# Spandan7724/Audio-Watermarking-Deep-Learning-Watermarks-for-Authenticating-Speech

Measured on AMD Instinct MI355X. Metric: 1-s@16kHz clips/sec (gen+det+loss fwd-bwd), higher is better.
Workload: dtype f32; 1 GPU; main16 train step: Generator+Detector+6 losses fwd-bwd + Adam, B=256 clips/GPU x 1 GPU, 1-s @ 16 kHz, message_bits=16 (BASELINE configs[2]); batch_per_gpu=256, global_batch=256, clip_len=16000, optimizer=fused flat Adam (wm_adam_step), parallelism=single

## Files before the change

audio-watermarking-deep-learning-watermarks-for-authenticating-speech_amd/csrc/lstm.hip:

```cpp
#include "wm_common.hpp"
#include <type_traits>
using namespace wm;

namespace {

#ifdef WM_STAMP
__device__ unsigned long long* g_lstm_stamp = nullptr;
#define LSTAMP(var, val) unsigned long long var; asm volatile("s_memtime %0\n\ts_waitcnt lgkmcnt(0)" : "=s"(var), "+v"(val))
#define LSTAMP_ACC(i, a, b) tm[i] += (b) - (a)
#else
#define LSTAMP(var, val)
#define LSTAMP_ACC(i, a, b)
#endif

__device__ __forceinline__ int gate_row(int np) { return (np & 3) * 64 + (np >> 2); }

typedef float v2f __attribute__((ext_vector_type(2)));
template <int K>
__device__ __forceinline__ float quad_bcast(float v) {
    constexpr int ctrl = K | (K << 2) | (K << 4) | (K << 6);
    return __int_as_float(__builtin_amdgcn_update_dpp(0, __float_as_int(v), ctrl, 0xf, 0xf, false));
}

__global__ __launch_bounds__(256) void lstm_xproj_kernel(const float* __restrict__ x, const float* __restrict__ w_ih,
// ... 613 lines not shown
#endif
    auto run_chunk = [&](const Buf& f, int t1) {
#pragma unroll
        for (int jj = 0; jj < CH; ++jj) {
            const int j = CH - 1 - jj, t = t1 - jj;
            if (t >= 0) {
                LSTAMP(ls0, dc);
                const float4 p = *reinterpret_cast<const float4*>(&part[pb][u][0]);
                const float act = f.ga[j];
                const float gi = quad_bcast<0>(act), gf = quad_bcast<1>(act), gg = quad_bcast<2>(act), go = quad_bcast<3>(act);
                const float tc = tanh_s(f.cc[j + 1]);
                const float cprev = (t >= 1) ? f.cc[j] : 0.f;
                const float S = is0 ? gg : (is1 ? cprev : (is2 ? gi : tc));
                const float D = is2 ? fmaf(-act, act, 1.f) : act * (1.f - act);
                const float M = S * D;
                const float K = go * fmaf(-tc, tc, 1.f);
                float dht = f.dh[j] + ((p.x + p.y) + (p.z + p.w));
                LSTAMP(ls1, dht);
                const float dct = fmaf(dht, K, dc);
                float da = (is3 ? dht : dct) * M;
                dc = dct * gf;
                LSTAMP(ls2, da);
                buf_store(sgb, da, vgb, (unsigned)t * 1024u);
                float Dd[4];
                rows_replicate(da, Dd);
                float psum = dot64_rowbcast(Dd, wt);
                LSTAMP(ls3, psum);
                part[pb ^ 1][lane][wave] = psum;
                pb ^= 1;
                LSTAMP(ls4, psum);
                __syncthreads();
                LSTAMP(ls5, dc);
                LSTAMP_ACC(0, ls0, ls1); LSTAMP_ACC(1, ls1, ls2); LSTAMP_ACC(2, ls2, ls3); LSTAMP_ACC(3, ls3, ls4); LSTAMP_ACC(4, ls4, ls5);
            }
        }
    };
    prefetch(A, T - 1);
    __syncthreads();
    for (int t1 = T - 1; t1 >= 0; t1 -= 2 * CH) {
        prefetch(Bf, t1 - CH);
        run_chunk(A, t1);
        prefetch(A, t1 - 2 * CH);
        run_chunk(Bf, t1 - CH);
    }
#ifdef WM_STAMP
    if (g_lstm_stamp && lane == 0) {
        unsigned long long* d = g_lstm_stamp + ((size_t)blockIdx.x * 4 + wave) * 6;
#pragma unroll
        for (int i = 0; i < 6; ++i) d[i] = tm[i];
    }
#endif
}

__global__ __launch_bounds__(512) void lstm_bwd_ws_kernel(float* __restrict__ gates, const float* __restrict__ cst,
                                                          const float* __restrict__ dh_out, const float* __restrict__ w_hh,
                                                          const float* __restrict__ x, const float* __restrict__ hseq,
                                                          float* __restrict__ partial, int T) {
    constexpr int CT = 32, PT = 36;
    extern __shared__ __align__(16) unsigned char smem_raw[];
    float* daT = reinterpret_cast<float*>(smem_raw);
    float (*part)[64][4] = reinterpret_cast<float (*)[64][4]>(daT + 2 * 256 * PT);
    const int b = blockIdx.x, tid = threadIdx.x, lane = tid & 63;
    const int wave = __builtin_amdgcn_readfirstlane(tid >> 6);
    float* out = partial + (size_t)b * (256 * 128 + 256);
    if (wave < 4) {
        __builtin_amdgcn_s_setprio(3);
        const int q = lane & 3, ul = lane >> 2, u = wave * 16 + ul, np = wave * 64 + lane;
        float wt[64];
#pragma unroll
        for (int j = 0; j < 64; ++j) wt[j] = w_hh[((j & 3) * 64 + wave * 16 + (j >> 2)) * 64 + lane];
        if (tid < 512 / 4) reinterpret_cast<float4*>(&part[0][0][0])[tid] = make_float4(0.f, 0.f, 0.f, 0.f);
        float dc = 0.f, dbs = 0.f;
        const wm_srd_t sgb = make_srd(gates + (size_t)b * T * 256, (size_t)T * 256 * sizeof(float));
        const wm_srd_t scb = make_srd(cst + (size_t)b * T * 64, (size_t)T * 64 * sizeof(float));
        const wm_srd_t sdh = make_srd(dh_out + (size_t)b * 64 * T, (size_t)64 * T * sizeof(float));
        const unsigned vgb = (unsigned)np * 4u, vcb = (unsigned)u * 4u, vdh = (unsigned)(u * T) * 4u;
        constexpr int CH = 8;
        struct Buf { float ga[CH], cc[CH + 1], dh[CH]; };
        Buf A, Bf;
        auto prefetch = [&](Buf& f, int t1) {
#pragma unroll
            for (int j = 0; j < CH; ++j) {
                const int t = max(t1 - CH + 1 + j, 0);
                f.ga[j] = buf_load(sgb, vgb, (unsigned)t * 1024u);
                f.dh[j] = buf_load(sdh, vdh, (unsigned)t * 4u);
            }
#pragma unroll
            for (int j = 0; j <= CH; ++j) f.cc[j] = buf_load(scb, vcb, (unsigned)max(t1 - CH + j, 0) * 256u);
        };
        const bool is0 = q == 0, is1 = q == 1, is2 = q == 2, is3 = q == 3;
        int pb = 0;
        auto run_chunk = [&](const Buf& f, int t1) {
            float dav[CH];
#pragma unroll
            for (int jj = 0; jj < CH; ++jj) {
                const int j = CH - 1 - jj, t = t1 - jj;
                const float4 p = *reinterpret_cast<const float4*>(&part[pb][u][0]);
                const float act = f.ga[j];
                const float gi = quad_bcast<0>(act), gf = quad_bcast<1>(act), gg = quad_bcast<2>(act), go = quad_bcast<3>(act);
                const float tc = tanh_s(f.cc[j + 1]);
                const float cprev = (t >= 1) ? f.cc[j] : 0.f;
                const float S = is0 ? gg : (is1 ? cprev : (is2 ? gi : tc));
                const float D = is2 ? fmaf(-act, act, 1.f) : act * (1.f - act);
                const float M = S * D;
                const float K = go * fmaf(-tc, tc, 1.f);
                const float dht = f.dh[j] + ((p.x + p.y) + (p.z + p.w));
                const float dct = fmaf(dht, K, dc);
                const float da = (is3 ? dht : dct) * M;
                dc = dct * gf;
                dav[j] = da;
                buf_store(sgb, da, vgb, (unsigned)t * 1024u);
                float Dd[4];
                rows_replicate(da, Dd);
                const float psum = dot64_rowbcast(Dd, wt);
                part[pb ^ 1][lane][wave] = psum;
                pb ^= 1;
                if (jj == CH - 1) {
                    const int t0 = t1 - (CH - 1);
                    float* d = daT + (((t0 >> 5) & 1) * 256 + np) * PT + (t0 & (CT - 1));
                    *reinterpret_cast<float4*>(d) = make_float4(dav[0], dav[1], dav[2], dav[3]);
                    *reinterpret_cast<float4*>(d + 4) = make_float4(dav[4], dav[5], dav[6], dav[7]);
                }
                dbs += da;
                __syncthreads();
            }
        };
        prefetch(A, T - 1);
        __syncthreads();
        for (int t1 = T - 1; t1 >= 0; t1 -= 2 * CH) {
            prefetch(Bf, t1 - CH);
            run_chunk(A, t1);
            prefetch(A, t1 - 2 * CH);
            run_chunk(Bf, t1 - CH);
        }
        out[256 * 128 + np] = dbs;
        return;
    }
    const int hw = wave - 4, half = lane >> 5, l31 = lane & 31;
    f32x16 acc[2][2][2];
#pragma unroll
    for (int i = 0; i < 8; ++i)
#pragma unroll
        for (int r = 0; r < 16; ++r) acc[i >> 2][(i >> 1) & 1][i & 1][r] = 0.f;
    const wm_srd_t sx = make_srd(x + (size_t)b * 64 * T, (size_t)64 * T * sizeof(float));
    const wm_srd_t sh = make_srd(hseq + (size_t)b * 64 * T, (size_t)64 * T * sizeof(float));
    float raw[8];
    auto load_raw = [&](int chunk, int u_) {
        const int ks = u_ >> 2, z = (u_ >> 1) & 1, ct = u_ & 1;
        const unsigned v = (unsigned)((32 * ct + l31) * T + 8 * half) * 4u;
        const int ts = chunk * CT + 16 * ks;
        if (z == 0) {
            const f32x4 a0 = buf_load4(sx, v, (unsigned)ts * 4u), a1 = buf_load4(sx, v, (unsigned)(ts + 4) * 4u);
            raw[0] = a0[0]; raw[1] = a0[1]; raw[2] = a0[2]; raw[3] = a0[3]; raw[4] = a1[0]; raw[5] = a1[1]; raw[6] = a1[2]; raw[7] = a1[3];
        } else {
#pragma unroll
            for (int e = 0; e < 8; ++e) {
                const int te = ts + e - 1;
                const float r_ = buf_load(sh, te < 0 ? v - 4u : v, (unsigned)max(te, 0) * 4u);
                raw[e] = (te < 0 && half == 0) ? 0.f : r_;
            }
        }
    };
    auto split8 = [&](const float (&v)[8], bf16x8 (&P)[3]) {
        unsigned w_[3][4];
#pragma unroll
        for (int i = 0; i < 4; ++i) split3_pair(v[2 * i], v[2 * i + 1], w_[0][i], w_[1][i], w_[2][i]);
#pragma unroll
        for (int p = 0; p < 3; ++p) P[p] = __builtin_bit_cast(bf16x8, make_uint4(w_[p][0], w_[p][1], w_[p][2], w_[p][3]));
    };
    bf16x8 Af[2][3], Bp[3];
    auto slot = [&](int chunk, int sl) {
        const int u_ = sl >> 2, k = sl & 3, ks = u_ >> 2, z = (u_ >> 1) & 1, ct = u_ & 1;
        if (k == 0) {
            if ((u_ & 3) == 0) {
#pragma unroll
                for (int rt = 0; rt < 2; ++rt) {
                    const float* src = daT + ((chunk & 1) * 256 + 64 * hw + 32 * rt + l31) * PT + 16 * ks + 8 * half;
                    const float4 a0 = *reinterpret_cast<const float4*>(src), a1 = *reinterpret_cast<const float4*>(src + 4);
                    const float v[8] = {a0.x, a0.y, a0.z, a0.w, a1.x, a1.y, a1.z, a1.w};
                    split8(v, Af[rt]);
                }
            }
            split8(raw, Bp);
            if (u_ < 7) load_raw(chunk, u_ + 1); else load_raw(max(chunk - 1, 0), 0);
            return;
        }
        constexpr int PA[6] = {1, 0, 2, 0, 1, 0}, PB[6] = {1, 2, 0, 1, 0, 0};
#pragma unroll
        for (int i = 0; i < 4; ++i) {
            const int m = 4 * (k - 1) + i, rt = m / 6, j = m % 6;
            acc[z][rt][ct] = __builtin_amdgcn_mfma_f32_32x32x16_bf16(Af[rt][PA[j]], Bp[PB[j]], acc[z][rt][ct], 0, 0, 0);
        }
    };
    const int nch = T / CT;
    load_raw(nch - 1, 0);
    __syncthreads();
    for (int c = nch - 1; c >= 0; --c) {
        const bool work = c + 1 < nch;
#pragma unroll
        for (int sl = 0; sl < CT; ++sl) {
            if (work) slot(c + 1, sl);
            __syncthreads();
        }
    }
#pragma unroll
    for (int sl = 0; sl < CT; ++sl) slot(0, sl);
#pragma unroll
    for (int z = 0; z < 2; ++z)
#pragma unroll
        for (int rt = 0; rt < 2; ++rt)
#pragma unroll
            for (int ct = 0; ct < 2; ++ct)
#pragma unroll
                for (int r = 0; r < 16; ++r)
                    out[(64 * hw + 32 * rt + mfma_row(r, half)) * 128 + 64 * z + 32 * ct + l31] = acc[z][rt][ct][r];
}

__global__ __launch_bounds__(256) void lstm_bwd_fused_kernel(float* __restrict__ gates, const float* __restrict__ cst,
                                                             const float* __restrict__ dh_out, const float* __restrict__ w_hh,
                                                             const float* __restrict__ w_ih, float* __restrict__ dx, int T) {
    constexpr int HS = WM_LSTM_HS, CHK = 32, PITCH = 72, NP = 3, PDP = 33;
    constexpr int DIMG = NP * CHK * PITCH;
    extern __shared__ __align__(16) unsigned char smem_raw[];
    unsigned short* Dab = reinterpret_cast<unsigned short*>(smem_raw);
    float* Pd = reinterpret_cast<float*>(Dab + 2 * 4 * DIMG);
    float* das = Pd + 4 * 64 * PDP;
    float* part = das + 4 * 64;
    const int b = blockIdx.x, tid = threadIdx.x, lane = tid & 63, wave = tid >> 6, half = lane >> 5, l31 = lane & 31;
    const int q = lane & 3, ul = lane >> 2, u = wave * 16 + ul, np = wave * 64 + lane;
    v2f wt[32];
#pragma unroll
    for (int j = 0; j < 64; j += 2)
        wt[j / 2] = v2f{w_hh[((j & 3) * 64 + wave * 16 + (j >> 2)) * 64 + lane],
                        w_hh[(((j + 1) & 3) * 64 + wave * 16 + ((j + 1) >> 2)) * 64 + lane]};
    bf16x8 Wt[2][4][NP];
#pragma unroll
    for (int mt = 0; mt < 2; ++mt)
#pragma unroll
        for (int ks = 0; ks < 4; ++ks) {
            float v[8];
#pragma unroll
            for (int j = 0; j < 8; ++j) v[j] = w_ih[gate_row(wave * 64 + 16 * ks + 8 * half + j) * 64 + mt * 32 + l31];
            unsigned a[4], m[4], l[4];
#pragma unroll
            for (int j = 0; j < 4; ++j) split3_pair(v[2 * j], v[2 * j + 1], a[j], m[j], l[j]);
            Wt[mt][ks][0] = __builtin_bit_cast(bf16x8, make_uint4(a[0], a[1], a[2], a[3]));
            Wt[mt][ks][1] = __builtin_bit_cast(bf16x8, make_uint4(m[0], m[1], m[2], m[3]));
            Wt[mt][ks][2] = __builtin_bit_cast(bf16x8, make_uint4(l[0], l[1], l[2], l[3]));
        }
    if (tid < 128) reinterpret_cast<float4*>(part)[tid] = make_float4(0.f, 0.f, 0.f, 0.f);
    float dc = 0.f;
    float* gb = gates + (size_t)b * T * 256 + np;
    const float* cb = cst + (size_t)b * T * 64 + u;
    const float* dhb = dh_out + ((size_t)b * 64 + u) * T;

    constexpr int CH = 8;
    struct Buf { float ga[CH], cc[CH + 1], dh[CH]; };
    Buf A, Bf;
    auto prefetch = [&](Buf& f, int t1) {
// ... 541 lines not shown
    if (g_lstm_fwd_ws) {
        static wm::DevOnce donew[2];
        if (int rc = wm::lds_opt_in(reinterpret_cast<const void*>(lstm_fwd_ws_kernel<true>), lds, donew[0])) return rc;
        if (int rc = wm::lds_opt_in(reinterpret_cast<const void*>(lstm_fwd_ws_kernel<false>), lds, donew[1])) return rc;
        if (gates && cst) hipLaunchKernelGGL(lstm_fwd_ws_kernel<true>, dim3(B), dim3(512), lds, stream, x, w_ih, b_ih, b_hh, w_hh, hout, gates, cst, T, LstmTailArgs<false>{});
        else hipLaunchKernelGGL(lstm_fwd_ws_kernel<false>, dim3(B), dim3(512), lds, stream, x, w_ih, b_ih, b_hh, w_hh, hout, gates, cst, T, LstmTailArgs<false>{});
        WM_CHECK_LAUNCH();
        return 0;
    }
    if (gates && cst) hipLaunchKernelGGL(lstm_fwd_fused_kernel<true>, dim3(B), dim3(256), lds, stream, x, w_ih, b_ih, b_hh, w_hh, hout, gates, cst, T);
    else hipLaunchKernelGGL(lstm_fwd_fused_kernel<false>, dim3(B), dim3(256), lds, stream, x, w_ih, b_ih, b_hh, w_hh, hout, gates, cst, T);
    WM_CHECK_LAUNCH();
    return 0;
}

int wm_lstm_fwd_tail(const float* xres, const float* y2, const float* sc2, const float* sh2, float* out, void* mask, const float* w_ih,
                     const float* b_ih, const float* b_hh, const float* w_hh, float* hout, float* gates, float* cst, int B, int T,
                     hipStream_t stream) {
    if (B <= 0 || T < 32 || (T & 31) || !xres || !y2 || !sc2 || !sh2 || !out) return (int)hipErrorInvalidValue;
    constexpr size_t lds = (size_t)2 * 32 * 257 * sizeof(float) + (size_t)3 * 32 * 72 * 2 + 128 * sizeof(float);
    static wm::DevOnce done[2];
    if (int rc = wm::lds_opt_in(reinterpret_cast<const void*>(lstm_fwd_ws_kernel<true, true>), lds, done[0])) return rc;
    if (int rc = wm::lds_opt_in(reinterpret_cast<const void*>(lstm_fwd_ws_kernel<false, true>), lds, done[1])) return rc;
    const LstmTailArgs<true> tl{y2, sc2, sh2, out, reinterpret_cast<unsigned*>(mask)};
    if (gates && cst) hipLaunchKernelGGL((lstm_fwd_ws_kernel<true, true>), dim3(B), dim3(512), lds, stream, xres, w_ih, b_ih, b_hh, w_hh, hout, gates, cst, T, tl);
    else hipLaunchKernelGGL((lstm_fwd_ws_kernel<false, true>), dim3(B), dim3(512), lds, stream, xres, w_ih, b_ih, b_hh, w_hh, hout, gates, cst, T, tl);
    WM_CHECK_LAUNCH();
    return 0;
}

int wm_lstm_bwd(float* gates, const float* cst, const float* dh_out, const float* w_hh, int B, int T, hipStream_t stream) {
    hipLaunchKernelGGL(lstm_bwd_kernel, dim3(B), dim3(256), 0, stream, gates, cst, dh_out, w_hh, T);
    WM_CHECK_LAUNCH();
    return 0;
}

int wm_lstm_bwd_fused(float* gates, const float* cst, const float* dh_out, const float* w_hh, const float* w_ih, float* dx,
                      int B, int T, hipStream_t stream) {
    if ((T & 3) || T < 4) return (int)hipErrorInvalidValue;
    constexpr size_t lds = (size_t)2 * 4 * 3 * 32 * 72 * 2 + (size_t)(4 * 64 * 33 + 4 * 64 + 2 * 64 * 4) * sizeof(float);
    static wm::DevOnce done;
    if (int rc = wm::lds_opt_in(reinterpret_cast<const void*>(lstm_bwd_fused_kernel), lds, done)) return rc;
    hipLaunchKernelGGL(lstm_bwd_fused_kernel, dim3(B), dim3(256), lds, stream, gates, cst, dh_out, w_hh, w_ih, dx, T);
    WM_CHECK_LAUNCH();
    return 0;
}

int wm_lstm_bwd_wgrad(float* gates, const float* cst, const float* dh_out, const float* w_hh, const float* x, const float* h,
                      float* partial, float* dw_ih, float* dw_hh, float* db_ih, float* db_hh, int B, int T, int accumulate,
                      hipStream_t stream) {
    if (B <= 0 || (T & 31) || T < 64) return (int)hipErrorInvalidValue;
    constexpr size_t lds = (size_t)(2 * 256 * 36 + 2 * 64 * 4) * sizeof(float);
    static wm::DevOnce done;
    if (int rc = wm::lds_opt_in(reinterpret_cast<const void*>(lstm_bwd_ws_kernel), lds, done)) return rc;
    hipLaunchKernelGGL(lstm_bwd_ws_kernel, dim3(B), dim3(512), lds, stream, gates, cst, dh_out, w_hh, x, h, partial, T);
    WM_CHECK_LAUNCH();
    hipLaunchKernelGGL(lstm_wgrad_reduce_kernel, dim3(kWgradSlab / 64), dim3(512), 0, stream, (const float*)partial, B,
                       dw_ih, dw_hh, db_ih, db_hh, accumulate);
    WM_CHECK_LAUNCH();
    return 0;
}

static int g_lstm_dx_bf = 1;
int wm_set_lstm_dx_bf16x6(int on, hipStream_t) { g_lstm_dx_bf = on ? 1 : 0; return 0; }

int wm_lstm_dx(const float* da, const float* w_ih, float* dx, int B, int T, hipStream_t stream) {
    const int ntiles = B * ((T + 63) / 64);
    if (g_lstm_dx_bf) {
        constexpr size_t ldsb = (size_t)3 * 64 * 264 * 2;
        static wm::DevOnce doneb;
        if (int rc = wm::lds_opt_in(reinterpret_cast<const void*>(lstm_dx_bf_kernel), ldsb, doneb)) return rc;
        hipLaunchKernelGGL(lstm_dx_bf_kernel, dim3(ntiles < kNumCU ? ntiles : kNumCU), dim3(256), ldsb, stream, da, w_ih, dx, B, T);
        WM_CHECK_LAUNCH();
        return 0;
    }
    constexpr size_t lds = (size_t)(256 * 64 + 64 * 257) * sizeof(float);
    static wm::DevOnce done;
    if (int rc = wm::lds_opt_in(reinterpret_cast<const void*>(lstm_dx_kernel), lds, done)) return rc;
    hipLaunchKernelGGL(lstm_dx_kernel, dim3(ntiles < kNumCU ? ntiles : kNumCU), dim3(256), lds, stream, da, w_ih, dx, B, T);
    WM_CHECK_LAUNCH();
    return 0;
}

int wm_lstm_wgrad(const float* da, const float* x, const float* h, float* partial, float* dw_ih, float* dw_hh,
                  float* db_ih, float* db_hh, int B, int T, int accumulate, hipStream_t stream) {
    int grid;
    if (g_lstm_dx_bf) {
        constexpr size_t ldsb = (size_t)(3 * 32 * 264 + 3 * 128 * 40) * 2;
        static wm::DevOnce doneb;
        if (int rc = wm::lds_opt_in(reinterpret_cast<const void*>(lstm_wgrad_bf_kernel), ldsb, doneb)) return rc;
        const int ntiles = B * ((T + 31) / 32);
        grid = ntiles < kNumCU ? ntiles : kNumCU;
        hipLaunchKernelGGL(lstm_wgrad_bf_kernel, dim3(grid), dim3(256), ldsb, stream, da, x, h, partial, B, T);
    } else {
        constexpr size_t lds = (size_t)(64 * 256 + 128 * 67) * sizeof(float);
        static wm::DevOnce done;
        if (int rc = wm::lds_opt_in(reinterpret_cast<const void*>(lstm_wgrad_kernel), lds, done)) return rc;
        const int ntiles = B * ((T + 63) / 64);
        grid = ntiles < kNumCU ? ntiles : kNumCU;
        hipLaunchKernelGGL(lstm_wgrad_kernel, dim3(grid), dim3(256), lds, stream, da, x, h, partial, B, T);
    }
    WM_CHECK_LAUNCH();
    hipLaunchKernelGGL(lstm_wgrad_reduce_kernel, dim3(kWgradSlab / 64), dim3(512), 0, stream, (const float*)partial, grid,
                       dw_ih, dw_hh, db_ih, db_hh, accumulate);
    WM_CHECK_LAUNCH();
    return 0;
}

}
```

audio-watermarking-deep-learning-watermarks-for-authenticating-speech_amd/ops.py:

```python
from __future__ import annotations

import contextlib
import math
import os

import torch

from ._lib import lib

NCU = 256
BN_EPS = 1e-5
BN_MOMENTUM = 0.1


def _stream():
    return torch.cuda.current_stream().cuda_stream


def _p(t):
    return None if t is None else t.data_ptr()


def _chk(t: torch.Tensor, name: str, ndim: int | None = None, dtype=torch.float32) -> torch.Tensor:
    if not isinstance(t, torch.Tensor):
# ... 210 lines not shown

def set_pair_fold(on: bool):
    set_switch("pair_fold", on)


def set_resblock_one_launch(on: bool):
    set_switch("one_launch_eval", on)


def conv_bf16x6() -> bool:
    return _CONV["bf16x6"]


def pack_w64_bf(w: torch.Tensor, mode: int) -> torch.Tensor:
    wpb = torch.empty(3 * 3 * 4096, dtype=torch.int16, device=w.device)
    lib.wm_pack_w64_bf(_p(w), _p(wpb), mode, _stream())
    return wpb


def set_conv7_f16x3(on: bool):
    set_switch("conv7_f16x3", on)


def pack_w64_h7(w: torch.Tensor, mode: int) -> torch.Tensor:
    wph = torch.empty(2 * 7 * 4096 + 4, dtype=torch.int16, device=w.device)
    lib.wm_pack_w64_h7(_p(w), _p(wph), mode, _stream())
    return wph


def set_lstm_fwd_wave_specialised(on: bool):
    set_switch("lstm_fwd_ws", on)


def set_lstm_bwd_wave_specialised(on: bool):
    set_switch("lstm_bwd_ws", on)


_HEADS = {"tail_in_head": os.environ.get("WM_TAIL_IN_HEAD", "1") == "1"}


def set_tail_in_head(on: bool):
    _HEADS["tail_in_head"] = bool(on)


def read_tail_in_consumer(environ) -> bool:
    return environ.get("WM_TAIL_IN_CONSUMER", "1") == "1"


_TAILC = {"on": read_tail_in_consumer(os.environ)}


def set_tail_in_consumer(on: bool):
    _TAILC["on"] = bool(on)


def _tail_in_consumer_launches(x, lstm: bool = False) -> bool:
    ok = (_TAILC["on"] and x.is_cuda and x.dim() == 3 and x.shape[-1] % 128 == 0 and _CONV["bf16x6"] and _CONV["fwd_f16x3"]
          and _CONV["schedule"] == 2)
    return bool(ok and (not lstm or (_LSTM["fused"] and _LSTM["fwd_ws"])))


def tail_in_consumer_applies(x, lstm: bool = False) -> bool:
    return _tail_in_consumer_launches(x, lstm) and bool(pair_node_applies(x))


def set_gconv_f16x3(on: bool):
    set_switch("gconv_f16x3", on)


_GMAX = {}


def _note_gmax(t: torch.Tensor, maxes: torch.Tensor, per_clip: bool = False):
    import weakref
    if len(_GMAX) > 256:
        _GMAX.clear()
    _GMAX[id(t)] = (weakref.ref(t), t._version, maxes, per_clip)


def _noted(t: torch.Tensor, pop: bool):
    e = _GMAX.pop(id(t), None) if pop else _GMAX.get(id(t))
    return e if e is not None and e[0]() is t and e[1] == t._version else None


def gscale_of(g: torch.Tensor, log2_target: float = 12.0) -> torch.Tensor:
    e = _noted(g, pop=True)
    if e is not None:
        gsc = _f32(2, device=g.device)
        lib.wm_gscale_from_max(_p(e[2]), e[2].numel(), float(log2_target), _p(gsc), _stream())
        return gsc
    return gscale_absmax(g, log2_target)


_ZPOOL = {"buf": None, "used": 0}


def zeroed_slots(n: int, device) -> torch.Tensor:
    p = _ZPOOL
    if p["buf"] is None or p["buf"].device != torch.device(device) or p["used"] + n > p["buf"].numel():
        p["buf"], p["used"] = torch.zeros(max(1 << 16, n), dtype=torch.float32, device=device), 0
    s = p["buf"][p["used"]:p["used"] + n]
    p["used"] += n
    return s


def amax_per_clip(x: torch.Tensor) -> torch.Tensor:
# ... 392 lines not shown
        else:
            d = torch.empty_like(logits)
            lib.wm_bce_bwd(_p(logits), _p(message), _p(gl), _p(gb), _p(d), message.shape[0], R, T, NO, st)
            d += g_logits
            lib.wm_headN_bwd(_p(d), _p(out), _p(hw), _p(dout), _p(part), _p(dhw), _p(dhb), R, T, NO, 0, st)
        dmid, grads2, fout = _resblock_bwd_fused(s2_, True, dout, fold=(s1_[3], s1_[2]))
        dx, grads1, _ = _resblock_bwd_fused(s1_, True, dmid, pre=fout)
        return (dx, None) + grads1 + (None,) * 6 + grads2 + (None,) * 6 + (dhw, dhb)


class LSTMFn(GradAwareFunction):

    @staticmethod
    def forward(ctx, x, w_ih, w_hh, b_ih, b_hh):
        need_grad = wants_grad(ctx)
        h, saved = _lstm_fwd(x, w_ih, w_hh, b_ih, b_hh, need_grad)
        if need_grad:
            ctx.gdst = _gdst(w_ih, w_hh, b_ih, b_hh)
            ctx.save_for_backward(*saved)
        return h

    @staticmethod
    def backward(ctx, dh):
        saved = ctx.saved_tensors
        _single_backward(ctx, "LSTMFn")
        return _lstm_bwd(saved, ctx.gdst, dh)


def _lstm_fwd(x, w_ih, w_hh, b_ih, b_hh, need_grad, tail=None):
    if tail is not None:
        xres, y2, sc2, sh2, mask = tail
        x = torch.empty_like(xres)
    x = _frames(x, "LSTM input", 64)
    B, _, T = x.shape
    dev, st = x.device, _stream()
    h = torch.empty_like(x)
    release_deferred_wgrads()
    cst = _f32(B, T, 64, device=dev) if need_grad else None
    if tail is not None:
        gates = _f32(B, T, 256, device=dev) if need_grad else None
        lib.wm_lstm_fwd_tail(_p(xres), _p(y2), _p(sc2), _p(sh2), _p(x), _p(mask), _p(w_ih), _p(b_ih), _p(b_hh), _p(w_hh), _p(h),
                             _p(gates), _p(cst), B, T, st)
    elif _LSTM["fused"] and T >= 8:
        gates = _f32(B, T, 256, device=dev) if need_grad else None
        lib.wm_lstm_fwd_fused(_p(x), _p(w_ih), _p(b_ih), _p(b_hh), _p(w_hh), _p(h), _p(gates), _p(cst), B, T, st)
    else:
        xp = _f32(B, T, 256, device=dev)
        lib.wm_lstm_xproj(_p(x), _p(w_ih), _p(b_ih), _p(b_hh), _p(xp), B, T, st)
        gates = xp if need_grad else None
        lib.wm_lstm_fwd(_p(xp), _p(w_hh), _p(h), _p(gates), _p(cst), B, T, st)
    return h, ((x, h, gates, cst, w_ih, w_hh) if need_grad else None)


def _lstm_bwd(saved, gdst, dh):
    x, h, gates, cst, w_ih, w_hh = saved
    dh = dh.contiguous()
    B, _, T = x.shape
    dev, st = x.device, _stream()
    dx = torch.empty_like(x)
    release_deferred_wgrads()
    dst, acc, launch = _wgrad_dst(gdst, dev, w_ih.shape, w_hh.shape, (256,), (256,))
    if _LSTM["bwd_ws"] and not _LSTM["bwd_fused"] and T % 32 == 0 and T >= 64:
        part = _f32(B * (256 * 128 + 256), device=dev)
        lib.wm_lstm_bwd_wgrad(_p(gates), _p(cst), _p(dh), _p(w_hh), _p(x), _p(h), _p(part), *map(_p, dst), B, T, int(acc), st)
        lib.wm_lstm_dx(_p(gates), _p(w_ih), _p(dx), B, T, st)
        return (dx,) + ((None,) * 4 if acc else dst)
    if _LSTM["bwd_fused"]:
        lib.wm_lstm_bwd_fused(_p(gates), _p(cst), _p(dh), _p(w_hh), _p(w_ih), _p(dx), B, T, st)
    else:
        lib.wm_lstm_bwd(_p(gates), _p(cst), _p(dh), _p(w_hh), B, T, st)
        lib.wm_lstm_dx(_p(gates), _p(w_ih), _p(dx), B, T, st)

    def wg():
        part = _f32(NCU * (256 * 128 + 256), device=dev)
        lib.wm_lstm_wgrad(_p(gates), _p(x), _p(h), _p(part), *map(_p, dst), B, T, int(acc), _stream())
    launch((gates, x, h), wg)
    return (dx,) + ((None,) * 4 if acc else dst)


class EncoderLSTMFn(GradAwareFunction):

    @staticmethod
    def forward(ctx, x, *args):
        p1, p2, (w_ih, w_hh, b_ih, b_hh) = args[:14], args[14:28], args[28:32]
        want = wants_grad(ctx)
        _, first, second = _pair_fwd(x, p1, p2, True, want, tail=False)
        mid, y2, cst = second[0], second[2], second[4]
        mask = _tail_mask(mid, want)
        h, lsaved = _lstm_fwd(None, w_ih, w_hh, b_ih, b_hh, want, tail=(mid, y2, cst[4], cst[5], mask))
        if want:
            ctx.gdst = _gdst(w_ih, w_hh, b_ih, b_hh)
            ctx.save_for_backward(*(first + second[:3] + (mask,) + second[4:] + lsaved))
        return h

    @staticmethod
    def backward(ctx, dh):
        sv = ctx.saved_tensors
        _single_backward(ctx, "EncoderLSTMFn")
        s1_, s2_ = sv[:9], sv[9:18]
        lgrads = _lstm_bwd(sv[18:], ctx.gdst, dh)
        dmid, grads2, fout = _resblock_bwd_fused(s2_, True, lgrads[0], fold=(s1_[3], s1_[2]))
        dx, grads1, _ = _resblock_bwd_fused(s1_, True, dmid, pre=fout)
        return (dx,) + grads1 + (None,) * 6 + grads2 + (None,) * 6 + lgrads[1:]


_CHECK_INDEX = {"mode": {"1": "sync", "0": "off"}.get(os.environ.get("WM_CHECK_INDEX", "1"), os.environ.get("WM_CHECK_INDEX", "sync")),
                "pending": []}


def set_index_check(mode):
    _CHECK_INDEX["mode"] = {True: "sync", False: "off"}.get(mode, mode)
    if _CHECK_INDEX["mode"] not in ("sync", "deferred", "off"):
        raise ValueError("index check mode must be 'sync', 'deferred' or 'off'")


@contextlib.contextmanager
def index_check_mode(mode=None):
    prev = _CHECK_INDEX["mode"]
    set_index_check(("deferred" if prev == "sync" else prev) if mode is None else mode)
    try:
        yield
    finally:
        _CHECK_INDEX["mode"] = prev


def index_check() -> str:
    return _CHECK_INDEX["mode"]


def check_message_ids(wait=True, what="an earlier Generator call"):
    keep = []
    for ev, host, nrows in _CHECK_INDEX["pending"]:
        if not wait and not ev.query():
            keep.append((ev, host, nrows))
            continue
        ev.synchronize()
        if int(host[0]) != 0:
            _CHECK_INDEX["pending"] = []
            raise IndexError(f"message id out of range for an embedding table of {nrows} rows (deferred check of {what})")
    _CHECK_INDEX["pending"] = keep


def drop_pending_message_checks():
    _CHECK_INDEX["pending"] = []


def _note_index_error(err, nrows):
    mode = _CHECK_INDEX["mode"]
    if mode == "off":
        return
    if mode == "sync":
        if int(err.item()) != 0:
            raise IndexError(f"message id out of range for an embedding table of {nrows} rows")
# ... 1150 lines not shown
```

include/wm_hip.h:

```cpp
#ifndef WM_HIP_H
#define WM_HIP_H

#ifdef __cplusplus
extern "C" {
#endif

typedef struct ihipStream_t* wm_stream_t;


int wm_pack_w64(const float* w, float* wp, int KW, int mode, wm_stream_t stream);

int wm_conv64(const float* x, const float* x2, const float* wp, const float* pa, const float* pb, const float* pc,
              const float* bias, const float* e1, const float* ea, const float* eb, float* y, float* stats,
              int B, int T, int KW, int pro, int epi, wm_stream_t stream);

int wm_pack_w64_bf(const float* w, void* wpb, int mode, wm_stream_t stream);
int wm_set_conv_bf_schedule(int schedule, wm_stream_t stream);
int wm_conv64_bf(const float* x, const float* x2, const void* wpb, const float* pa, const float* pb, const float* pc,
                 const float* bias, const float* e1, const float* ea, const float* eb, float* y, float* stats,
                 int B, int T, int pro, int epi, int arith, wm_stream_t stream);
int wm_conv64_bf_tail(const float* x, const float* y2, const void* wpb_h, const float* sc2, const float* sh2, const float* bias,
                      float* out, void* mask, float* y, float* stats, int B, int T, wm_stream_t stream);

int wm_pack_w64_bf_scaled(const float* w, const float* row_scale, void* wpb, wm_stream_t stream);
// ... 30 lines not shown
                   float* running_mean, float* running_var, long long* num_batches_tracked, float momentum, float eps,
                   float* scale, float* shift, float* save_mean, float* save_invstd, wm_stream_t stream);
int wm_bn_eval_scale_shift(const float* gamma, const float* beta, const float* running_mean, const float* running_var,
                           float eps, float* scale, float* shift, wm_stream_t stream);
int wm_bn_add_relu(const float* x, const float* y2, const float* scale, const float* shift, float* out, int B, int T,
                   wm_stream_t stream);
int wm_relu_bwd_reduce(const float* g, const float* out, const float* y2, float* dz, float* partial, int B, int T,
                       wm_stream_t stream);
int wm_bn_add_relu_mask(const float* x, const float* y2, const float* scale, const float* shift, float* out, void* mask, int B, int T,
                        wm_stream_t stream);
int wm_relu_bwd_reduce_mask(const float* g, const void* mask, const float* y2, float* dz, float* partial, float* dzmax, int B, int T,
                            wm_stream_t stream);
int wm_bn_bwd_finalize(const float* partials, int nparts, double count, const float* gamma, const float* save_mean,
                       const float* save_invstd, float* A, float* Bc, float* Cc, float* dgamma, float* dbeta,
                       int accumulate, int eval_mode, const float* dzmax, int nmax, float* gscale, wm_stream_t stream);

int wm_stem_fwd(const float* s, const float* w, const float* bias, float* y, int B, int T, wm_stream_t stream);
int wm_stem_bwd(const float* g, const float* s, const float* w, float* ds, float* partial, float* dw, float* db, int B,
                int T, int nds, int accumulate, wm_stream_t stream);
int wm_head1_fwd(const float* x, const float* w, const float* bias, float* y, int B, int T, wm_stream_t stream);
int wm_head1_bwd(const float* g, const float* x, const float* w, float* dx, float* partial, float* dw, float* db, int B,
                 int T, int accumulate, wm_stream_t stream);
int wm_headN_fwd(const float* x, const float* w, const float* bias, float* y, int B, int T, int NO, wm_stream_t stream);
int wm_headN_bwd(const float* g, const float* x, const float* w, float* dx, float* partial, float* dw, float* db, int B,
                 int T, int NO, int accumulate, wm_stream_t stream);
int wm_head1_tail_fwd(const float* x, const float* y2, const float* scale, const float* shift, const float* w, const float* bias,
                      float* out, void* mask, float* y, int B, int T, wm_stream_t stream);
int wm_headN_tail_fwd(const float* x, const float* y2, const float* scale, const float* shift, const float* w, const float* bias,
                      const long long* message, int B, float* partial, float* loc_out, float* bce_out, float* out, void* mask,
                      float* logits, int R, int T, int NO, wm_stream_t stream);
int wm_headN_bwd_bce(const float* logits, const long long* message, const float* g_loc, const float* g_bce, const float* x,
                     const float* w, float* dx, float* partial, float* dw, float* db, int B, int R, int T, int NO, int accumulate,
                     wm_stream_t stream);

int wm_lstm_xproj(const float* x, const float* w_ih, const float* b_ih, const float* b_hh, float* xp, int B, int T,
                  wm_stream_t stream);
int wm_lstm_fwd(const float* xp, const float* w_hh, float* hout, float* gates, float* cst, int B, int T, wm_stream_t stream);
int wm_lstm_fwd_fused(const float* x, const float* w_ih, const float* b_ih, const float* b_hh, const float* w_hh,
                      float* hout, float* gates, float* cst, int B, int T, wm_stream_t stream);
int wm_set_lstm_fwd_wave_specialised(int on, wm_stream_t stream);
int wm_lstm_fwd_tail(const float* xres, const float* y2, const float* sc2, const float* sh2, float* out, void* mask, const float* w_ih,
                     const float* b_ih, const float* b_hh, const float* w_hh, float* hout, float* gates, float* cst, int B, int T,
                     wm_stream_t stream);
int wm_lstm_bwd(float* gates, const float* cst, const float* dh_out, const float* w_hh, int B, int T, wm_stream_t stream);
int wm_lstm_dx(const float* da, const float* w_ih, float* dx, int B, int T, wm_stream_t stream);
int wm_set_lstm_dx_bf16x6(int on, wm_stream_t stream);
int wm_lstm_bwd_fused(float* gates, const float* cst, const float* dh_out, const float* w_hh, const float* w_ih, float* dx,
                      int B, int T, wm_stream_t stream);
int wm_lstm_wgrad(const float* da, const float* x, const float* h, float* partial, float* dw_ih, float* dw_hh,
                  float* db_ih, float* db_hh, int B, int T, int accumulate, wm_stream_t stream);
int wm_lstm_bwd_wgrad(float* gates, const float* cst, const float* dh_out, const float* w_hh, const float* x, const float* h,
                      float* partial, float* dw_ih, float* dw_hh, float* db_ih, float* db_hh, int B, int T, int accumulate,
                      wm_stream_t stream);

int wm_embed_gather(const float* table, const long long* message, float* vec, int B, int nrows, int* err, wm_stream_t stream);
int wm_embed_scatter_add(float* dtable, const long long* message, const float* dvec, int B, int nrows, wm_stream_t stream);
int wm_rowsum(const float* x, float* out, int rows, int T, wm_stream_t stream);

int wm_postproc_fwd(const float* d_in, const float* taps, int ntaps, float thr, float max_rms, float eps, int stages,
                    float* f_out, float* d_out, float* stats, int B, int T, wm_stream_t stream);
int wm_postproc_bwd(const float* g, const float* f_in, const float* stats, const float* taps, int ntaps, float thr,
                    float max_rms, int stages, float* d_raw, int B, int T, wm_stream_t stream);

int wm_mel_loss(const float* clean, const float* wm, const float* fb, const int* klo, const int* khi, const int* mlo,
                float* gframes, float* partial, float* loss_out, float* dsig, int B, int T, wm_stream_t stream);
int wm_loud_loss(const float* clean, const float* wm, float thresh, float* gframes, float* partial, float* loss_out,
                 float* dsig, int B, int T, wm_stream_t stream);
int wm_hf_penalty(const float* delta, int kcut, float* gframes, float* partial, float* loss_out, float* dsig, int B, int T,
                  wm_stream_t stream);

int wm_bce_fwd(const float* logits, const long long* message, float* partial, float* loc_out, float* bce_out, int B, int R,
               int T, int NO, wm_stream_t stream);
int wm_bce_bwd(const float* logits, const long long* message, const float* g_loc, const float* g_bce, float* dlogits, int B,
               int R, int T, int NO, wm_stream_t stream);
int wm_l1_fwd(const float* x, float* partial, float* out, long long n, wm_stream_t stream);
int wm_l1_bwd(const float* x, const float* g, float* dx, long long n, wm_stream_t stream);
int wm_adam_step(float* p, const float* g, float* m, float* v, long long n, double lr, double beta1, double beta2, double eps,
                 int step, wm_stream_t stream);

int wm_gconv(const float* x, const float* wp, const float* bias, const float* vec, const float* res, float* y, int NB,
             int Cin, int Lin, int K, int S, int P, int Mtot, int Nout, int st, int shp, int Cout, int Lout, int act,
             const float* x2, int Cin1, int nph, wm_stream_t stream);
int wm_gconv_h(const float* x, const void* wph, const float* bias, const float* vec, const float* res, float* y, int NB,
               int Cin, int Lin, int K, int S, int P, int Mtot, int Nout, int st, int shp, int Cout, int Lout, int act,
               const float* x2, int Cin1, int nph, const float* gscale, float* ymax, int per_clip, wm_stream_t stream);
int wm_gconv_pack_h(const float* wp, void* wph, float* scratch, int Cin, int K, int Mtot, wm_stream_t stream);
int wm_gconv_pack_h_conv(const float* w, void* wph, int Cout, int Cin, int K, int mode, wm_stream_t stream);
int wm_gwgrad_plan(int NB, int Ca, int Cb, int La, int K, long long* slab_floats, wm_stream_t stream);
int wm_gwgrad(const float* A, const float* Bx, float* G, float* dbias, float* slab, int NB, int Ca, int Cb, int La, int Lb,
              int K, int P, long long b_clip_stride, int remap, int r1, int r2, int accumulate, wm_stream_t stream);
int wm_gather_taps(const float* x, float* y, int NB, int C, int Lin, int K, int S, int P, int Lout, int order, wm_stream_t stream);
int wm_elu_bwd(const float* g, const float* y, float* dz, long long n, wm_stream_t stream);
int wm_channel_sum(const float* x, float* out, float* partial, int NB, int C, int L, int accumulate, wm_stream_t stream);
int wm_rowsum_any(const float* x, float* out, int rows, int L, wm_stream_t stream);
int wm_rows_scatter_add(float* dtable, const long long* idx, const float* dvec, int Bn, int dim, int nrows, wm_stream_t stream);
int wm_permute_acl(const float* x, float* y, int A, int C, int L, wm_stream_t stream);
int wm_lstm_seq_fwd(float* xp, const float* whh, float* hs, float* cs, int T, int H, int B, int save, wm_stream_t stream);
int wm_lstm_seq_bwd(float* gates, const float* cs, const float* dout, const float* whhT, float* dc, int T, int H, int B,
                    wm_stream_t stream);

int wm_resample_plan(int P, int Q, int width, int W, long long* tile_periods, wm_stream_t stream);
int wm_resample(const float* x, const float* taps, const int* first, float* y, int C, long long N, int P, int Q, int width, int W,
                long long L, long long total, wm_stream_t stream);

int wm_resample_add(const float* d, const float* taps, const int* first, const float* x, float* out, float* up, int C, long long N,
                    long long Nd, int P, int Q, int width, int W, wm_stream_t stream);
// ... 53 lines not shown
```

Before: 5502 clips/s.

## Fuse LSTM input-gradient dx GEMM into warp-specialised backward wgrad kernel

Adds a DX template variant of the warp-specialised LSTM backward kernel. The worker waves that already run the weight-gradient MFMA slots now also compute dx = da·W_ih from the da tiles held in LDS, using a bf16x6 split of W_ih staged in LDS and scratch. In the fused path the per-timestep da store back to global memory and the separate lstm_dx launch are dropped, removing a full re-read of da. The cost is extra LDS, more register pressure and more work interleaved between barriers. It is enabled by default through an environment flag when async mode is off.

```diff
diff --git a/audio-watermarking-deep-learning-watermarks-for-authenticating-speech_amd/csrc/lstm.hip b/audio-watermarking-deep-learning-watermarks-for-authenticating-speech_amd/csrc/lstm.hip
--- a/audio-watermarking-deep-learning-watermarks-for-authenticating-speech_amd/csrc/lstm.hip
+++ b/audio-watermarking-deep-learning-watermarks-for-authenticating-speech_amd/csrc/lstm.hip
@@ -689,10 +689,12 @@
 #endif
 }
 
+template <bool DX>
 __global__ __launch_bounds__(512) void lstm_bwd_ws_kernel(float* __restrict__ gates, const float* __restrict__ cst,
                                                           const float* __restrict__ dh_out, const float* __restrict__ w_hh,
                                                           const float* __restrict__ x, const float* __restrict__ hseq,
-                                                          float* __restrict__ partial, int T) {
+                                                          float* __restrict__ partial, const float* __restrict__ w_ih,
+                                                          float* __restrict__ dx, int T) {
     constexpr int CT = 32, PT = 36;
     extern __shared__ __align__(16) unsigned char smem_raw[];
     float* daT = reinterpret_cast<float*>(smem_raw);
@@ -746,7 +748,7 @@
                 const float da = (is3 ? dht : dct) * M;
                 dc = dct * gf;
                 dav[j] = da;
-                buf_store(sgb, da, vgb, (unsigned)t * 1024u);
+                if constexpr (!DX) buf_store(sgb, da, vgb, (unsigned)t * 1024u);
                 float Dd[4];
                 rows_replicate(da, Dd);
                 const float psum = dot64_rowbcast(Dd, wt);
@@ -829,9 +831,82 @@
             acc[z][rt][ct] = __builtin_amdgcn_mfma_f32_32x32x16_bf16(Af[rt][PA[j]], Bp[PB[j]], acc[z][rt][ct], 0, 0, 0);
         }
     };
+    bf16x8* const wl = reinterpret_cast<bf16x8*>(smem_raw + (2 * 256 * PT + 2 * 64 * 4) * sizeof(float)) + hw * (16 * 2 * 64) + lane;
+    const wm_srd_t swg = make_srd(out + hw * (64 * 128), (size_t)16 * 64 * 16);
+    const wm_srd_t sdx = make_srd(DX ? dx + ((size_t)b * 64 + hw * 32) * T : nullptr, (size_t)32 * T * sizeof(float));
+    const unsigned vdx = (unsigned)(4 * half * T + l31) * 4u;
+    bf16x8 Bd[3], A2[2];
+    f32x16 dacc;
+    if constexpr (DX) {
+        if (hw < 2) {
+#pragma unroll 2
+            for (int ks = 0; ks < 16; ++ks) {
+                float v[8];
+#pragma unroll
+                for (int j = 0; j < 8; ++j) v[j] = w_ih[gate_row(16 * ks + 8 * half + j) * 64 + hw * 32 + l31];
+                bf16x8 P[3];
+                split8(v, P);
+                wl[(2 * ks) * 64] = P[0];
+                wl[(2 * ks + 1) * 64] = P[1];
+                buf_store4(swg, __builtin_bit_cast(f32x4, P[2]), (unsigned)lane * 16u, (unsigned)ks * 1024u);
+            }
+        }
+    }
+    auto load_a2 = [&](int ks) { return __builtin_bit_cast(bf16x8, buf_load4(swg, (unsigned)lane * 16u, (unsigned)ks * 1024u)); };
+    auto dx_gather = [&](int chunk, int ks) {
+        const float* src = daT + ((chunk & 1) * 256 + 16 * ks + 8 * half) * PT + l31;
+        float v[8];
+#pragma unroll
+        for (int j = 0; j < 8; ++j) v[j] = src[j * PT];
+        split8(v, Bd);
+    };
+    auto dx_mul = [&](int ks, const bf16x8& a2) {
+        const bf16x8 Ap[3] = {wl[(2 * ks) * 64], wl[(2 * ks + 1) * 64], a2};
+        dacc = mfma_bf16x6(Ap, Bd, dacc);
+    };
+    auto dx_slot = [&](int chunk, int sl) {
+        if (hw >= 2) return;
+        const int g = sl >> 2, k = sl & 3;
+        if (sl == 0) {
+#pragma unroll
+            for (int r = 0; r < 16; ++r) dacc[r] = 0.f;
+        }
+        if (k == 1) dx_gather(chunk, 2 * g);
+        if (k == 2) {
+            dx_mul(2 * g, A2[0]);
+            dx_gather(chunk, 2 * g + 1);
+        }
+        if (k == 3) {
+            dx_mul(2 * g + 1, A2[1]);
+            A2[0] = load_a2((2 * g + 2) & 15);
+            A2[1] = load_a2((2 * g + 3) & 15);
+            if (sl == CT - 1) {
+#pragma unroll
+                for (int r = 0; r < 16; ++r) buf_store(sdx, dacc[r], vdx, (unsigned)(mfma_row(r, 0) * T + chunk * CT) * 4u);
+            }
+        }
+    };
+    if constexpr (DX) {
+        if (hw < 2) {
+            A2[0] = load_a2(0);
+            A2[1] = load_a2(1);
+        }
+    }
     const int nch = T / CT;
     load_raw(nch - 1, 0);
     __syncthreads();
+    if constexpr (DX) {
+#pragma unroll 1
+        for (int sl = 0; sl < CT; ++sl) __syncthreads();
+        for (int c = nch - 2; c >= 0; --c) {
+#pragma unroll
+            for (int sl = 0; sl < CT; ++sl) {
+                slot(c + 1, sl);
+                dx_slot(c + 1, sl);
+                __syncthreads();
+            }
+        }
+    } else
     for (int c = nch - 1; c >= 0; --c) {
         const bool work = c + 1 < nch;
 #pragma unroll
@@ -841,7 +916,11 @@
         }
     }
 #pragma unroll
-    for (int sl = 0; sl < CT; ++sl) slot(0, sl);
+    for (int sl = 0; sl < CT; ++sl) {
+        slot(0, sl);
+        if constexpr (DX) dx_slot(0, sl);
+    }
+    if constexpr (DX) asm volatile("s_waitcnt vmcnt(0)" ::: "memory");
 #pragma unroll
     for (int z = 0; z < 2; ++z)
 #pragma unroll
@@ -1489,8 +1568,9 @@
     if (B <= 0 || (T & 31) || T < 64) return (int)hipErrorInvalidValue;
     constexpr size_t lds = (size_t)(2 * 256 * 36 + 2 * 64 * 4) * sizeof(float);
     static wm::DevOnce done;
-    if (int rc = wm::lds_opt_in(reinterpret_cast<const void*>(lstm_bwd_ws_kernel), lds, done)) return rc;
-    hipLaunchKernelGGL(lstm_bwd_ws_kernel, dim3(B), dim3(512), lds, stream, gates, cst, dh_out, w_hh, x, h, partial, T);
+    if (int rc = wm::lds_opt_in(reinterpret_cast<const void*>(lstm_bwd_ws_kernel<false>), lds, done)) return rc;
+    hipLaunchKernelGGL(lstm_bwd_ws_kernel<false>, dim3(B), dim3(512), lds, stream, gates, cst, dh_out, w_hh, x, h, partial,
+                       (const float*)nullptr, (float*)nullptr, T);
     WM_CHECK_LAUNCH();
     hipLaunchKernelGGL(lstm_wgrad_reduce_kernel, dim3(kWgradSlab / 64), dim3(512), 0, stream, (const float*)partial, B,
                        dw_ih, dw_hh, db_ih, db_hh, accumulate);
@@ -1515,6 +1595,28 @@
     static wm::DevOnce done;
     if (int rc = wm::lds_opt_in(reinterpret_cast<const void*>(lstm_dx_kernel), lds, done)) return rc;
     hipLaunchKernelGGL(lstm_dx_kernel, dim3(ntiles < kNumCU ? ntiles : kNumCU), dim3(256), lds, stream, da, w_ih, dx, B, T);
+    WM_CHECK_LAUNCH();
+    return 0;
+}
+
+int wm_lstm_bwd_wgrad_dx(const float* gates, const float* cst, const float* dh_out, const float* w_hh, const float* w_ih,
+                         const float* x, const float* h, float* partial, float* dw_ih, float* dw_hh, float* db_ih, float* db_hh,
+                         float* dx, int B, int T, int accumulate, hipStream_t stream) {
+    if (B <= 0 || (T & 31) || T < 64 || !dx || !w_ih || (reinterpret_cast<uintptr_t>(partial) & 15)) return (int)hipErrorInvalidValue;
+    if (!g_lstm_dx_bf) {
+        if (int rc = wm_lstm_bwd_wgrad(const_cast<float*>(gates), cst, dh_out, w_hh, x, h, partial, dw_ih, dw_hh, db_ih, db_hh, B, T,
+                                       accumulate, stream))
+            return rc;
+        return wm_lstm_dx(gates, w_ih, dx, B, T, stream);
+    }
+    constexpr size_t lds = (size_t)(2 * 256 * 36 + 2 * 64 * 4) * sizeof(float) + (size_t)2 * 16 * 2 * 64 * 16;
+    static wm::DevOnce done;
+    if (int rc = wm::lds_opt_in(reinterpret_cast<const void*>(lstm_bwd_ws_kernel<true>), lds, done)) return rc;
+    hipLaunchKernelGGL(lstm_bwd_ws_kernel<true>, dim3(B), dim3(512), lds, stream, const_cast<float*>(gates), cst, dh_out, w_hh, x, h,
+                       partial, w_ih, dx, T);
+    WM_CHECK_LAUNCH();
+    hipLaunchKernelGGL(lstm_wgrad_reduce_kernel, dim3(kWgradSlab / 64), dim3(512), 0, stream, (const float*)partial, B,
+                       dw_ih, dw_hh, db_ih, db_hh, accumulate);
     WM_CHECK_LAUNCH();
     return 0;
 }
diff --git a/audio-watermarking-deep-learning-watermarks-for-authenticating-speech_amd/ops.py b/audio-watermarking-deep-learning-watermarks-for-authenticating-speech_amd/ops.py
--- a/audio-watermarking-deep-learning-watermarks-for-authenticating-speech_amd/ops.py
+++ b/audio-watermarking-deep-learning-watermarks-for-authenticating-speech_amd/ops.py
@@ -286,6 +286,17 @@
 
 def set_tail_in_consumer(on: bool):
     _TAILC["on"] = bool(on)
+
+
+def read_lstm_dx_in_bwd(environ) -> bool:
+    return environ.get("WM_LSTM_DX_IN_BWD", "1") == "1"
+
+
+_LSTM_DX = {"in_bwd": read_lstm_dx_in_bwd(os.environ)}
+
+
+def set_lstm_dx_in_bwd(on: bool):
+    _LSTM_DX["in_bwd"] = bool(on)
 
 
 def _tail_in_consumer_launches(x, lstm: bool = False) -> bool:
@@ -784,7 +795,7 @@
     return h, ((x, h, gates, cst, w_ih, w_hh) if need_grad else None)
 
 
-def _lstm_bwd(saved, gdst, dh):
+def _lstm_bwd(saved, gdst, dh, dx_inside=False):
     x, h, gates, cst, w_ih, w_hh = saved
     dh = dh.contiguous()
     B, _, T = x.shape
@@ -794,6 +805,10 @@
     dst, acc, launch = _wgrad_dst(gdst, dev, w_ih.shape, w_hh.shape, (256,), (256,))
     if _LSTM["bwd_ws"] and not _LSTM["bwd_fused"] and T % 32 == 0 and T >= 64:
         part = _f32(B * (256 * 128 + 256), device=dev)
+        if dx_inside and not _ASYNC["on"]:
+            lib.wm_lstm_bwd_wgrad_dx(_p(gates), _p(cst), _p(dh), _p(w_hh), _p(w_ih), _p(x), _p(h), _p(part), *map(_p, dst), _p(dx),
+                                     B, T, int(acc), st)
+            return (dx,) + ((None,) * 4 if acc else dst)
         lib.wm_lstm_bwd_wgrad(_p(gates), _p(cst), _p(dh), _p(w_hh), _p(x), _p(h), _p(part), *map(_p, dst), B, T, int(acc), st)
         lib.wm_lstm_dx(_p(gates), _p(w_ih), _p(dx), B, T, st)
         return (dx,) + ((None,) * 4 if acc else dst)
@@ -830,7 +845,7 @@
         sv = ctx.saved_tensors
         _single_backward(ctx, "EncoderLSTMFn")
         s1_, s2_ = sv[:9], sv[9:18]
-        lgrads = _lstm_bwd(sv[18:], ctx.gdst, dh)
+        lgrads = _lstm_bwd(sv[18:], ctx.gdst, dh, dx_inside=_LSTM_DX["in_bwd"])
         dmid, grads2, fout = _resblock_bwd_fused(s2_, True, lgrads[0], fold=(s1_[3], s1_[2]))
         dx, grads1, _ = _resblock_bwd_fused(s1_, True, dmid, pre=fout)
         return (dx,) + grads1 + (None,) * 6 + grads2 + (None,) * 6 + lgrads[1:]
diff --git a/include/wm_hip.h b/include/wm_hip.h
--- a/include/wm_hip.h
+++ b/include/wm_hip.h
@@ -106,6 +106,9 @@
 int wm_lstm_bwd_wgrad(float* gates, const float* cst, const float* dh_out, const float* w_hh, const float* x, const float* h,
                       float* partial, float* dw_ih, float* dw_hh, float* db_ih, float* db_hh, int B, int T, int accumulate,
                       wm_stream_t stream);
+int wm_lstm_bwd_wgrad_dx(const float* gates, const float* cst, const float* dh_out, const float* w_hh, const float* w_ih,
+                         const float* x, const float* h, float* partial, float* dw_ih, float* dw_hh, float* db_ih, float* db_hh,
+                         float* dx, int B, int T, int accumulate, wm_stream_t stream);
 
 int wm_embed_gather(const float* table, const long long* message, float* vec, int B, int nrows, int* err, wm_stream_t stream);
 int wm_embed_scatter_add(float* dtable, const long long* message, const float* dvec, int B, int nrows, wm_stream_t stream);
```

Result: faster. 5648 clips/s, median of 6 (+2.6%).
